# TNO-MPC/protocols.distributed_keygen

Measured on NVIDIA B200. Metric: threshold decrypts/sec (2048-bit N), higher is better.
Workload: dtype u32 limbs (exact integer)

## Files before the change

### protocols/distributed_keygen_b200/csrc/dkg_coop.cuh

```cuda
#pragma once
#include <cuda_runtime.h>
#include <stdint.h>

#include "dkg_coop_params.h"
#include "dkg_mont.cuh"

namespace dkg {

namespace coop {

using sa = uint32_t;
__device__ __forceinline__ sa saddr(const void* p) { return (sa)__cvta_generic_to_shared(p); }

template <int K>
struct NoIO {
  static constexpr int VW = 2;
  struct Prefetch {};
  __device__ __forceinline__ void prefetch_load(const Prefetch&, int, uint32_t (&)[K]) const {}
};

template <int K>
__device__ __forceinline__ void lds(uint32_t (&r)[K], sa p) {
  if constexpr (K % 4 == 0) {
#pragma unroll
// ... 3 lines not shown
  } else {
#pragma unroll
    for (int v = 0; v < K / 2; ++v)
      asm volatile("ld.shared.v2.u32 {%0, %1}, [%2];" : "=r"(r[2 * v]), "=r"(r[2 * v + 1]) : "r"(p + 8u * v) : "memory");
  }
}
template <int K>
__device__ __forceinline__ void sts(sa p, const uint32_t (&r)[K]) {
#pragma unroll
  for (int v = 0; v < K / 2; ++v)
    asm volatile("st.shared.v2.u32 [%0], {%1, %2};" :: "r"(p + 8u * v), "r"(r[2 * v]), "r"(r[2 * v + 1]) : "memory");
}
__device__ __forceinline__ uint32_t lds1(sa p) {
  uint32_t v;
  asm volatile("ld.shared.u32 %0, [%1];" : "=r"(v) : "r"(p) : "memory");
  return v;
}

struct LanePlan {
  int d, i0, i1, p0, p1, p2, rounds, ndiag;
  __device__ __forceinline__ void load(const CoopPlanTable& t, int lane) {
    d = t.d[lane]; i0 = t.i0[lane]; i1 = t.i1[lane];
    p0 = t.partner[0][lane]; p1 = t.partner[1][lane]; p2 = t.partner[2][lane];
    rounds = t.rounds; ndiag = t.ndiag;
  }
};

template <int K, int NS>
__device__ __forceinline__ void product(uint32_t (&e)[NS][2 * K + 2], const LanePlan& lp, int lane, const sa (&X)[NS],
                                        const sa (&Y)[NS], const sa (&X2)[NS], const sa (&Y2)[NS]) {
  ColAcc<K> a[NS];
#pragma unroll
  for (int s = 0; s < NS; ++s) {
#pragma unroll
    for (int p = 0; p < 2 * K + 2; ++p) e[s][p] = 0;
    acc_load<K>(a[s], e[s]);
    acc_clear_side<K>(a[s]);
  }
  const NoIO<K> io;
  const typename NoIO<K>::Prefetch pf;
  for (int i = lp.i0; i < lp.i1; ++i) {
    uint32_t xb[NS][K], yb[NS][K];
    const uint32_t ox = (uint32_t)(i * K * 4), oy = (uint32_t)((lp.d - i) * K * 4);
#pragma unroll
    for (int s = 0; s < NS; ++s) { lds<K>(xb[s], X[s] + ox); lds<K>(yb[s], Y[s] + oy); }
#pragma unroll
    for (int s = 0; s < NS; ++s) block_mac<K>(a[s], xb[s], yb[s], io, pf);
#pragma unroll
    for (int s = 0; s < NS; ++s) {
      if (X2[s] != 0) {
        lds<K>(xb[s], X2[s] + ox);
        lds<K>(yb[s], Y2[s] + oy);
        block_mac<K>(a[s], xb[s], yb[s], io, pf);
      }
    }
  }
  __syncwarp();
#pragma unroll
  for (int s = 0; s < NS; ++s) acc_merge<K>(a[s], e[s]);
  for (int r = 0; r < lp.rounds; ++r) {
    const int src = r == 0 ? lp.p0 : (r == 1 ? lp.p1 : lp.p2);
    const int from = src >= 0 ? src : lane;
    const uint32_t m = src >= 0 ? 0xffffffffu : 0u;
#pragma unroll
    for (int s = 0; s < NS; ++s) {
      uint32_t t[2 * K + 2];
#pragma unroll
      for (int k = 0; k < 2 * K + 2; ++k) t[k] = __shfl_sync(kCoopFull, e[s][k], from) & m;
      add_cc(e[s][0], t[0]);
#pragma unroll
// ... 729 lines not shown
```

### protocols/distributed_keygen_b200/csrc/dkg_modexp.cuh

```cuda
#pragma once
#include <cuda_runtime.h>
#include "dkg_mont.cuh"
#include "dkg_modexp_params.h"

namespace dkg {

template <int K> struct VecSel { using T = uint2; static constexpr int VW = 2; };
#define DKG_VEC4(K_) template <> struct VecSel<K_> { using T = uint4; static constexpr int VW = 4; };
DKG_VEC4(4) DKG_VEC4(8) DKG_VEC4(12) DKG_VEC4(16) DKG_VEC4(20) DKG_VEC4(24) DKG_VEC4(28) DKG_VEC4(32)
#undef DKG_VEC4

__device__ __forceinline__ void unpack(const uint4& v, uint32_t* r) { r[0] = v.x; r[1] = v.y; r[2] = v.z; r[3] = v.w; }
__device__ __forceinline__ void unpack(const uint2& v, uint32_t* r) { r[0] = v.x; r[1] = v.y; }
__device__ __forceinline__ void pack(uint4& v, const uint32_t* r) { v = make_uint4(r[0], r[1], r[2], r[3]); }
__device__ __forceinline__ void pack(uint2& v, const uint32_t* r) { v = make_uint2(r[0], r[1]); }

__device__ __forceinline__ void lds_vec(uint4& v, uint32_t saddr) {
  asm volatile("ld.shared.v4.u32 {%0, %1, %2, %3}, [%4];" : "=r"(v.x), "=r"(v.y), "=r"(v.z), "=r"(v.w) : "r"(saddr) : "memory");
}
__device__ __forceinline__ void lds_vec(uint2& v, uint32_t saddr) {
  asm volatile("ld.shared.v2.u32 {%0, %1}, [%2];" : "=r"(v.x), "=r"(v.y) : "r"(saddr) : "memory");
}
__device__ __forceinline__ void sts_vec(uint32_t saddr, const uint4& v) {
  asm volatile("st.shared.v4.u32 [%0], {%1, %2, %3, %4};" :: "r"(saddr), "r"(v.x), "r"(v.y), "r"(v.z), "r"(v.w) : "memory");
// ... 97 lines not shown
    for (int q = 0; q < KV; q++) { V v; ldg_vec(v, Qg + (size_t)(i * KV + q) * 32); unpack(v, &r[q * VW]); }
  }
  struct Prefetch { const char* base; };
  __device__ __forceinline__ Prefetch prefetch_desc(int kind, int blk) const {
    Prefetch d;
    const bool xkind = kind == PAIR_XX || kind == PAIR_XX2 || kind == PAIR_SX2;
    const bool from_shared = xkind && !x_global();
    const bool none = !(xkind || kind == PAIR_XY || kind == PAIR_NQ || kind == PAIR_SY2);
    unsigned long long sgen;
    const uint32_t sbase = none ? ss : xs;
    asm("cvta.shared.u64 %0, %1;" : "=l"(sgen) : "l"((unsigned long long)(sbase + (uint32_t)((none ? 0 : blk) * KV) * 32u * VB)));
    const V* g = kind == PAIR_XY ? Y : (kind == PAIR_SY2 ? Y2 : ((xkind && x_global()) ? this->xg_get() : Qg));
    const char* gb = reinterpret_cast<const char*>(g + (size_t)(blk * KV) * 32);
    d.base = (from_shared || none) ? reinterpret_cast<const char*>(sgen) : gb;
    return d;
  }
  __device__ __forceinline__ void prefetch_load(const Prefetch& d, int v, uint32_t (&r)[KP]) const {
    V val;
    ld_generic(val, d.base + (size_t)v * 32u * VB);
    unpack(val, &r[v * VW]);
  }
  __device__ __forceinline__ void load_n(int j, uint32_t (&r)[KP]) const {
#pragma unroll
    for (int q = 0; q < KV; q++) { V v; lds_vec(v, ns + (uint32_t)(j * KV + q) * NSTRIDE); unpack(v, &r[q * VW]); }
  }
  __device__ __forceinline__ void load_ninv(uint32_t (&r)[KP]) const {
#pragma unroll
    for (int q = 0; q < KV; q++) { V v; lds_vec(v, nis + (uint32_t)q * NSTRIDE); unpack(v, &r[q * VW]); }
  }
  __device__ __forceinline__ void store_q(int i, const uint32_t (&r)[KP]) const {
#pragma unroll
    for (int q = 0; q < KV; q++) { V v; pack(v, &r[q * VW]); stg_vec(Qg + (size_t)(i * KV + q) * 32, v); }
  }
  __device__ __forceinline__ void store_x(int i, const uint32_t (&r)[KP]) const {
    if (x_global()) {
#pragma unroll
      for (int q = 0; q < KV; q++) { V v; pack(v, &r[q * VW]); stg_vec(this->xg_get() + (size_t)(i * KV + q) * 32, v); }
      return;
    }
#pragma unroll
    for (int q = 0; q < KV; q++) { V v; pack(v, &r[q * VW]); sts_vec(xs + (uint32_t)(i * KV + q) * 32u * VB, v); }
  }
};


template <int VW>
__device__ __forceinline__ int sidx(int l) { return (l / VW) * 32 * VW + (l % VW); }

static __device__ __noinline__ uint32_t* mod_inverse_arrays(uint32_t* pu, uint32_t* pv, uint32_t* px1, uint32_t* px2,
                                                     const uint32_t* Ns, uint32_t n0inv, int Lp, uint32_t* bad_out) {
  uint32_t nz = 0;
  for (int l = 0; l < Lp; ++l) {
    pv[l * 32] = Ns[l];
    px1[l * 32] = (l == 0) ? 1u : 0u;
    px2[l * 32] = 0u;
    nz |= pu[l * 32];
  }
  int len = Lp;
  int guard = 64 * Lp + 64;
  while (nz != 0 && guard-- > 0) {
    uint32_t u0 = pu[0];
    while ((u0 & 1u) == 0) {
      const int tz = u0 ? __ffs(u0) - 1 : 32;
      uint32_t lo = u0;
      for (int l = 0; l < len; ++l) {
        const uint32_t hi = (l + 1 < len) ? pu[(l + 1) * 32] : 0u;
// ... 33 lines not shown
    }
    bool xlt = false;
    for (int l = Lp - 1; l >= 0; --l) {
      const uint32_t a = px1[l * 32], b = px2[l * 32];
      if (a != b) { xlt = a < b; break; }
    }
    const uint32_t addmask = xlt ? 0xffffffffu : 0u;
    int64_t c = 0;
    for (int l = 0; l < Lp; ++l) {
      const int64_t t = (int64_t)px1[l * 32] - (int64_t)px2[l * 32] + (int64_t)(Ns[l] & addmask) + c;
      px1[l * 32] = (uint32_t)t;
      c = t >> 32;
    }
    while (len > 1 && pu[(len - 1) * 32] == 0 && pv[(len - 1) * 32] == 0) --len;
  }
  uint32_t bad = pv[0] ^ 1u;
  for (int l = 1; l < Lp; ++l) bad |= pv[l * 32];
  *bad_out = bad ? 1u : 0u;
  return px2;
}

template <int K, int M>
__device__ uint32_t mod_inverse_lane(uint32_t* X, const uint32_t* Ns, uint32_t n0inv, uint32_t* g) {
  constexpr int VW = VecSel<K>::VW;
  constexpr int Lp = K * M;
  for (int l = 0; l < Lp; ++l) g[l * 32] = X[sidx<VW>(l)];
  uint32_t bad = 0;
  const uint32_t* r = mod_inverse_arrays(g, g + Lp * 32, g + 2 * Lp * 32, g + 3 * Lp * 32, Ns, n0inv, Lp, &bad);
  for (int l = 0; l < Lp; ++l) X[sidx<VW>(l)] = r[l * 32];
  return bad;
}

template <int K, int M, bool PLN, bool SCHED, bool XG>
__device__ __noinline__ void mont_call_rt(const WarpIO<K, M, PLN, SCHED, XG> io, const int mode) {
  mont_mul<K, M>(io, mode);
}
template <int K, int M, int MODE, bool PLN = false, bool SCHED = false, bool XG = false>
__device__ __forceinline__ void mont_call(const WarpIO<K, M, PLN, SCHED, XG>& io) {
  mont_call_rt<K, M, PLN, SCHED, XG>(io, MODE);
}
template <int M>
__device__ __forceinline__ void fill_schedule(uint32_t* tab) {
  const int n = sched_offset<M>(kSchedModes);
  for (int i = threadIdx.x; i < n; i += blockDim.x) tab[i] = sched_entry<M>(i);
}

template <int K, int M>
__global__ void __launch_bounds__(DKG_MAX_THREADS, 1) modexp_fixed_kernel(const ModexpParams p) {
  using V = typename VecSel<K>::T;
  constexpr int VW = VecSel<K>::VW;
  constexpr int Lp = K * M;
  constexpr int LV = Lp / VW;

  extern __shared__ __align__(16) unsigned char smem_raw[];
  uint32_t* Ns32 = reinterpret_cast<uint32_t*>(smem_raw);
  constexpr int UNI = ((Lp + K) * 4 + 15) / 16 * 16;
  const int lane = threadIdx.x & 31, warp = threadIdx.x >> 5, nwarps = blockDim.x >> 5;

  for (int i = threadIdx.x; i < Lp + K; i += blockDim.x) Ns32[i] = p.consts[i];
  __syncthreads();

  V* Xw = reinterpret_cast<V*>(smem_raw + UNI) + (size_t)warp * LV * 32;
  uint32_t* Xw32 = reinterpret_cast<uint32_t*>(Xw);
  const V* Ns = reinterpret_cast<const V*>(Ns32);
  const V* NIs = reinterpret_cast<const V*>(Ns32 + Lp);
  const V* ONEg = reinterpret_cast<const V*>(p.consts + Lp + K + Lp);
  const V* R2rep = reinterpret_cast<const V*>(p.consts + Lp + K + 3 * Lp) + lane;
  const V* ONErep = R2rep + (size_t)LV * 32;

  const unsigned gwarp = blockIdx.x * nwarps + warp;
  uint32_t* scratch32 = p.scratch + (size_t)gwarp * p.scratch_per_warp;
  V* tab = reinterpret_cast<V*>(scratch32);
// ... 116 lines not shown
```

### protocols/distributed_keygen_b200/csrc/dkg_mont.cuh

```cuda
#pragma once
#include "dkg_prims.cuh"

namespace dkg {

enum MontMode { MONT_MUL = 0, MONT_REDC = 1, MONT_SQR = 2, MONT_MUL2S = 3, MONT_MULADD = 4 };

#ifndef DKG_PIPE_BALLAST
#define DKG_PIPE_BALLAST 4096
#endif
DKG_HD uint32_t pipe_ballast(uint32_t a, uint32_t b) {
#if defined(__CUDA_ARCH__)
  float f = __uint_as_float(a);
  const float g = __uint_as_float(b);
#pragma unroll
  for (int q = 0; q < DKG_PIPE_BALLAST; q++) asm volatile("fma.rn.f32 %0, %0, %1, %1;" : "+f"(f) : "f"(g));
  return __float_as_uint(f);
#else
  return a ^ b;
#endif
}

template <int K> constexpr int kpad = K + (K & 1);
template <int K> constexpr int kodd0 = K + 1 - (K & 1);
template <int K> constexpr int kncE = (2 * K - kpad<K>) / 2 + 1;
// ... 22 lines not shown

struct PairDesc {
  int kind, xi, yi;
};

template <int K, class IO>
DKG_HD void block_mac(ColAcc<K>& a, const uint32_t (&x)[kpad<K>], uint32_t (&y)[kpad<K>], const IO& io,
                      const typename IO::Prefetch& pf) {
  static_assert(K >= 4, "K must be >= 4");
  constexpr int VW = IO::VW;
#pragma unroll
  for (int j = 0; j < K; j++) {
    {
      const int i0 = j & 1;
      const int last = ((K - 1 - i0) & 1) ? K - 2 : K - 1;
      mad_cc64(a.E[(i0 + j) / 2], x[i0], y[j]);
#pragma unroll
      for (int i = i0 + 2; i < last; i += 2) madc_cc64(a.E[(i + j) / 2], x[i], y[j]);
      madc_cc64_count(a.E[(last + j) / 2], x[last], y[j], a.CE[(last + j + 2 - kpad<K>) / 2]);
    }
    {
      const int i0 = (j & 1) ^ 1;
      const int last = ((K - 1 - i0) & 1) ? K - 2 : K - 1;
      mad_cc64(a.O[(i0 + j - 1) / 2], x[i0], y[j]);
#pragma unroll
      for (int i = i0 + 2; i < last; i += 2) madc_cc64(a.O[(i + j - 1) / 2], x[i], y[j]);
      madc_cc64_count(a.O[(last + j - 1) / 2], x[last], y[j], a.CO[(last + j + 2 - kodd0<K>) / 2]);
    }
    if ((j + 1) % VW == 0 || j == K - 1) io.prefetch_load(pf, j / VW, y);
  }
}

template <int K>
DKG_HD void acc_merge(ColAcc<K>& a, uint32_t (&e)[2 * K + 2]) {
  uint32_t o[2 * K - 2];
#pragma unroll
  for (int p = 0; p < K + 1; p++) unpack64(a.E[p], e[2 * p], e[2 * p + 1]);
#pragma unroll
  for (int p = 0; p < K - 1; p++) unpack64(a.O[p], o[2 * p], o[2 * p + 1]);
  add_cc(e[1], o[0]);
#pragma unroll
  for (int p = 1; p < 2 * K - 2; p++) addc_cc(e[p + 1], o[p]);
  addc_cc(e[2 * K - 1], 0);
  addc_cc(e[2 * K], 0);
  addc(e[2 * K + 1], 0);
#pragma unroll
  for (int p = K; p <= 2 * K; p++) {
    const bool even = ((p - kpad<K>) & 1) == 0;
    const uint32_t cnt = even ? a.CE[(p - kpad<K>) / 2] : a.CO[(p - kodd0<K>) / 2];
    if (p == K) add_cc(e[p], cnt); else addc_cc(e[p], cnt);
  }
  addc(e[2 * K + 1], 0);
  acc_clear_side<K>(a);
}

template <int K>
DKG_HD void acc_low(const ColAcc<K>& a, uint32_t (&tl)[K]) {
  uint32_t t[kpad<K>], o[kpad<K>];
#pragma unroll
  for (int p = 0; p < (K + 1) / 2; p++) unpack64(a.E[p], t[2 * p], t[2 * p + 1]);
#pragma unroll
  for (int p = 0; p < K / 2; p++) unpack64(a.O[p], o[2 * p], o[2 * p + 1]);
  add_cc(t[1], o[0]);
#pragma unroll
  for (int p = 2; p < K; p++) {
    if (p < K - 1) addc_cc(t[p], o[p - 1]); else addc(t[p], o[p - 1]);
  }
#pragma unroll
  for (int p = 0; p < K; p++) tl[p] = t[p];
}

template <int K>
DKG_HD void acc_load(ColAcc<K>& a, const uint32_t (&e)[2 * K + 2]) {
#pragma unroll
  for (int p = 0; p < K + 1; p++) a.E[p] = pack64(e[2 * p], e[2 * p + 1]);
}

template <int K, int XN>
DKG_HD void block_mul_lo(uint32_t (&r)[kpad<K>], const uint32_t (&x)[XN], const uint32_t (&y)[kpad<K>]) {
  static_assert(XN >= K, "x too short");
  uint32_t E[K + 1], O[K + 1];
#pragma unroll
  for (int i = 0; i < K + 1; i++) { E[i] = 0; O[i] = 0; }
#pragma unroll
  for (int j = 0; j < K; j++) {
    {
      const int i0 = j & 1;
#pragma unroll
      for (int i = i0; i + j <= K - 1; i += 2) {
        const int pos = i + j;
        if (pos <= K - 2) { if (i == i0) mad_cc(E[pos], E[pos + 1], x[i], y[j]); else madc_cc(E[pos], E[pos + 1], x[i], y[j]); }
        else { if (i == i0) mad_lo(E[pos], x[i], y[j]); else madc_lo(E[pos], x[i], y[j]); }
      }
    }
    {
      const int i0 = (j & 1) ^ 1;
#pragma unroll
      for (int i = i0; i + j <= K - 1; i += 2) {
        const int q = i + j - 1;
        if (q + 1 <= K - 2) { if (i == i0) mad_cc(O[q], O[q + 1], x[i], y[j]); else madc_cc(O[q], O[q + 1], x[i], y[j]); }
        else { if (i == i0) mad_lo(O[q], x[i], y[j]); else madc_lo(O[q], x[i], y[j]); }
      }
    }
  }
  r[0] = E[0];
  r[1] = E[1];
  add_cc(r[1], O[0]);
#pragma unroll
  for (int p = 2; p < K - 1; p++) { r[p] = E[p]; addc_cc(r[p], O[p - 1]); }
  r[K - 1] = E[K - 1];
  addc(r[K - 1], O[K - 2]);
  if (K & 1) r[K] = 0;
}

template <int M>
struct ColPlan {
  int lo = 0, span = 0, nxy = 0, nq = 0, total = 0, MODE = 0;
  DKG_HD constexpr ColPlan(int c, int mode) {
    MODE = mode;
    lo = c >= M ? c - M + 1 : 0;
    const int hi = c < M ? c : M - 1;
    span = hi - lo + 1;
    nxy = (MODE == MONT_MUL || MODE == MONT_MUL2S) ? span
          : (MODE == MONT_SQR ? span / 2 + (span & 1) : (MODE == MONT_MULADD ? 2 * span : 0));
    nq = (c < M ? c - 1 : M - 1) - lo + 1;
    total = nxy + nq + (c < M ? 1 : 0);
  }
  DKG_HD constexpr PairDesc at(int c, int t) const {
    PairDesc d{PAIR_NONE, 0, 0};
    if (t < nq) { d.kind = PAIR_NQ; d.yi = lo + t; d.xi = c - d.yi; }
    else if (t < nq + nxy) {
      const int u = t - nq;
      if (MODE == MONT_MULADD && u >= span) { d.kind = PAIR_SY2; d.xi = lo + (u - span); d.yi = c - d.xi; }
      else {
        d.xi = lo + u; d.yi = c - d.xi;
        d.kind = MODE == MONT_SQR ? (d.xi < d.yi ? PAIR_XX2 : PAIR_XX) : (MODE == MONT_MUL2S ? PAIR_SX2 : PAIR_XY);
      }
    } else d.kind = PAIR_QC;
    return d;
  }
};

DKG_HD uint32_t pack_desc(const PairDesc& d) { return (uint32_t)d.kind | ((uint32_t)d.xi << 8) | ((uint32_t)d.yi << 16); }
DKG_HD PairDesc unpack_desc(uint32_t w) {
  PairDesc d;
  d.kind = (int)(w & 0xffu); d.xi = (int)((w >> 8) & 0xffu); d.yi = (int)((w >> 16) & 0xffu);
  return d;
}
constexpr int kSchedModes = 5;
template <int M>
DKG_HD constexpr int sched_words(int mode) {
  int n = 1;
  for (int c = 0; c < 2 * M; ++c) n += ColPlan<M>(c, mode).total;
  return n;
}
template <int M>
DKG_HD constexpr int sched_offset(int mode) {
  int off = 0;
  for (int m = 0; m < mode; ++m) off += sched_words<M>(m);
  return off;
}
template <int M>
DKG_HD uint32_t sched_entry(int i) {
  for (int mode = 0; mode < kSchedModes; ++mode) {
    const int n = sched_words<M>(mode);
    if (i >= n) { i -= n; continue; }
    for (int c = 0; c < 2 * M; ++c) {
      const ColPlan<M> plan(c, mode);
      if (i < plan.total) return pack_desc(plan.at(c, i));
      i -= plan.total;
    }
    break;
  }
  PairDesc none;
  none.kind = PAIR_NONE; none.xi = 0; none.yi = 0;
  return pack_desc(none);
}

template <int K, int M, class IO>
DKG_HD void mont_mul(const IO& io, const int MODE) {
  using Plan = ColPlan<M>;
  ColAcc<K> a;
  uint32_t e[2 * K + 2];
  uint32_t Tc[K + 2];
#pragma unroll
  for (int i = 0; i < K + 2; i++) Tc[i] = 0;
  acc_clear_side<K>(a);

  auto sched = io.sched_begin(IO::SCHED ? sched_offset<M>(MODE) + 1 : 0);
  uint32_t sched_ahead = 0;
  if constexpr (IO::SCHED) sched_ahead = io.sched_word(sched, 0);

  constexpr int KP = kpad<K>;
  uint32_t xb[KP], yb[KP];
  {
    const PairDesc d = Plan(0, MODE).at(0, 0);
    if (d.kind == PAIR_XY) { io.load_x(d.xi, xb); io.load_y(d.yi, yb); }
    else if (d.kind == PAIR_XX) { io.load_x(d.xi, xb); io.load_x(d.yi, yb); }
    else if (d.kind == PAIR_SX2) { io.load_xs2(true, d.xi, xb); io.load_x(d.yi, yb); }
  }

  for (int c = 0; c < 2 * M; ++c) {
    const Plan plan(c, MODE);

#pragma unroll
    for (int p = 0; p < K + 2; p++) e[p] = Tc[p];
#pragma unroll
    for (int p = K + 2; p < 2 * K + 2; p++) e[p] = 0;

    if (MODE == MONT_REDC && c < M) {
      uint32_t tb[KP];
      io.load_x(c, tb);
      add_cc(e[0], tb[0]);
#pragma unroll
      for (int p = 1; p < K; p++) addc_cc(e[p], tb[p]);
#pragma unroll
      for (int p = K; p <= 2 * K; p++) addc_cc(e[p], 0);
      addc(e[2 * K + 1], 0);
    }
    if (MODE == MONT_SQR && (c & 1) == 0 && c >= 2) {
      const int j = c >> 1;
      const uint32_t mask = 0u - (io.x_top_limb(j - 1) >> 31);
      uint32_t tb[KP];
      io.load_x(j, tb);
      add_cc(e[0], tb[0] & mask);
#pragma unroll
      for (int p = 1; p < K; p++) addc_cc(e[p], tb[p] & mask);
#pragma unroll
      for (int p = K; p <= 2 * K; p++) addc_cc(e[p], 0);
      addc(e[2 * K + 1], 0);
    }
    const int t_quot = c < M ? plan.total - 1 : -1;
    int t = 0;
    while (t < plan.total) {
      if (t == 0) acc_load<K>(a, e);
      if (t == t_quot) {
        uint32_t tl[K];
        acc_low<K>(a, tl);
        io.load_ninv(yb);
        block_mul_lo<K>(xb, tl, yb);
        io.store_q(c, xb);
        io.load_n(0, yb);
      }
      int t_end = plan.total;
      if (t < t_quot) t_end = t_quot;
      for (; t < t_end; ++t) {
        PairDesc nx;
        if constexpr (IO::SCHED) {
          nx = unpack_desc(sched_ahead);
          sched = io.sched_next(sched);
          sched_ahead = io.sched_word(sched, 0);
        } else {
          nx.kind = PAIR_NONE; nx.xi = 0; nx.yi = 0;
          if (t + 1 < plan.total) nx = plan.at(c, t + 1);
          else if (c + 1 < 2 * M) {
            const Plan np(c + 1, MODE);
            if (np.total > 0) nx = np.at(c + 1, 0);
          }
        }
        block_mac<K>(a, xb, yb, io, io.prefetch_desc(nx.kind, nx.yi));
        if (nx.kind == PAIR_NQ) io.load_n(nx.xi, xb);
        else if (nx.kind == PAIR_XX2 || nx.kind == PAIR_SX2) io.load_xs2(nx.kind == PAIR_SX2, nx.xi, xb);
        else if (nx.kind != PAIR_QC && nx.kind != PAIR_NONE) io.load_xs(nx.kind == PAIR_SY2, nx.xi, xb);
      }
    }
    if (plan.total > 0) acc_merge<K>(a, e);

    if (c >= M) {
      uint32_t ob[KP];
#pragma unroll
      for (int p = 0; p < K; p++) ob[p] = e[p];
      if (K & 1) ob[K] = 0;
      io.store_x(c - M, ob);
    }
#pragma unroll
    for (int p = 0; p < K + 2; p++) Tc[p] = e[p + K];
  }

  if (io.never()) Tc[0] = pipe_ballast(Tc[0], Tc[1]);
  if (!io.any_lane(Tc[0])) return;
  const uint32_t mask = 0u - Tc[0];
  uint32_t borrow = 0;
  for (int b = 0; b < M; ++b) {
    uint32_t tb[kpad<K>], nb[kpad<K>];
    io.load_x(b, tb);
    io.load_n(b, nb);
#pragma unroll
    for (int p = 0; p < K; p++) {
      const uint64_t d = (uint64_t)tb[p] - (nb[p] & mask) - borrow;
      tb[p] = (uint32_t)d;
      borrow = (uint32_t)(d >> 63);
    }
    io.store_x(b, tb);
  }
}

template <int K, int M, class IO>
DKG_HD uint32_t geq_n(const IO& io) {
  uint32_t borrow = 0;
  for (int b = 0; b < M; ++b) {
    uint32_t xb[kpad<K>], nb[kpad<K>];
    io.load_x(b, xb);
    io.load_n(b, nb);
#pragma unroll
    for (int p = 0; p < K; p++) {
      const uint64_t d = (uint64_t)xb[p] - nb[p] - borrow;
      borrow = (uint32_t)(d >> 63);
    }
  }
  return borrow ^ 1u;
}

template <int K, int M, class IO>
DKG_HD void sub_n_masked(const IO& io, uint32_t mask) {
  uint32_t borrow = 0;
  for (int b = 0; b < M; ++b) {
    uint32_t xb[kpad<K>], nb[kpad<K>];
    io.load_x(b, xb);
    io.load_n(b, nb);
#pragma unroll
    for (int p = 0; p < K; p++) {
      const uint64_t d = (uint64_t)xb[p] - (nb[p] & mask) - borrow;
      xb[p] = (uint32_t)d;
      borrow = (uint32_t)(d >> 63);
    }
    io.store_x(b, xb);
  }
// ... 12 lines not shown
```

### protocols/distributed_keygen_b200/csrc/dkg_nsq.cuh

```cuda
#pragma once
#include "dkg_modexp.cuh"
#include "dkg_nsq_params_fwd.h"

namespace dkg {


template <int K, int M>
__device__ __forceinline__ void pair_fixup(typename VecSel<kpad<K>>::T* Bv, const typename VecSel<kpad<K>>::T* mq,
                                           const uint32_t* Ns, const uint32_t* Dneg) {
  constexpr int KP = kpad<K>;
  using V = typename VecSel<KP>::T;
  constexpr int VW = VecSel<KP>::VW;
  constexpr int LV = KP * M / VW;
  auto is_pad = [](int v, int k) -> bool { return (K & 1) && (v * VW + k) % KP == K; };
  uint32_t carry = 1;
  for (int v = 0; v < LV; ++v) {
    uint32_t bb[VW], mm[VW];
    unpack(Bv[v * 32], bb);
    unpack(mq[(size_t)v * 32], mm);
#pragma unroll
    for (int k = 0; k < VW; ++k) {
      if (is_pad(v, k)) { bb[k] = 0; continue; }
      const uint64_t s = (uint64_t)bb[k] + (uint32_t)~mm[k] + carry;
      bb[k] = (uint32_t)s;
      carry = (uint32_t)(s >> 32);
    }
    V o; pack(o, bb); Bv[v * 32] = o;
  }
  const uint32_t need = carry ^ 1u;
  if (__any_sync(0xffffffffu, need)) {
    const uint32_t mask = 0u - need;
    uint32_t c2 = 0;
    for (int v = 0; v < LV; ++v) {
      uint32_t bb[VW];
      unpack(Bv[v * 32], bb);
#pragma unroll
      for (int k = 0; k < VW; ++k) {
        if (is_pad(v, k)) continue;
        const uint64_t s = (uint64_t)bb[k] + (Dneg[v * VW + k] & mask) + c2;
        bb[k] = (uint32_t)s;
        c2 = (uint32_t)(s >> 32);
      }
      V o; pack(o, bb); Bv[v * 32] = o;
    }
    if (__any_sync(0xffffffffu, c2)) {
      const uint32_t mask2 = 0u - c2;
      uint32_t borrow = 0;
      for (int v = 0; v < LV; ++v) {
        uint32_t bb[VW];
        unpack(Bv[v * 32], bb);
#pragma unroll
        for (int k = 0; k < VW; ++k) {
          if (is_pad(v, k)) continue;
          const uint64_t d = (uint64_t)bb[k] - (Ns[v * VW + k] & mask2) - borrow;
          bb[k] = (uint32_t)d;
          borrow = (uint32_t)(d >> 63);
        }
        V o; pack(o, bb); Bv[v * 32] = o;
      }
    }
  }
}

template <int K, int M, class PairMul>
__device__ __forceinline__ uint32_t pair_invert(typename VecSel<kpad<K>>::T* Aw, typename VecSel<kpad<K>>::T* Bw,
                                                uint32_t* work, const uint32_t* U32, const uint32_t* Nd,
                                                const uint32_t* two_ab, const typename VecSel<kpad<K>>::T* R2Ar,
                                                const typename VecSel<kpad<K>>::T* R2Br, int lane, PairMul&& pair_mul) {
  constexpr int KP = kpad<K>;
  using V = typename VecSel<KP>::T;
  constexpr int VW = VecSel<KP>::VW;
  constexpr int Lp = KP * M, La = K * M, LV = Lp / VW, KVB = KP / VW;
  uint32_t* Aw32 = reinterpret_cast<uint32_t*>(Aw);
  uint32_t* Bw32 = reinterpret_cast<uint32_t*>(Bw);
  uint32_t* pu = work + lane;
  uint32_t* pv = pu + La * 32;
  V* slots = reinterpret_cast<V*>(work + 2 * Lp * 32);
  auto slot_a = [&](int s) -> V* { return slots + (size_t)s * 2 * LV * 32 + lane; };
  auto slot_b = [&](int s) -> V* { return slots + ((size_t)s * 2 + 1) * LV * 32 + lane; };
  auto sidx_of = [&](int l) -> int { const int sl = (l / K) * KP + l % K; return ((sl / VW) * 32 + lane) * VW + sl % VW; };
  for (int v = 0; v < LV; ++v) { slot_a(0)[(size_t)v * 32] = Aw[v * 32 + lane]; slot_b(0)[(size_t)v * 32] = Bw[v * 32 + lane]; }
  for (int l = 0; l < La; ++l) pu[l * 32] = Aw32[sidx_of(l)];
  uint32_t bad = 0;
  const uint32_t* g = mod_inverse_arrays(pu, pv, Aw32 + lane, Bw32 + lane, Nd, U32[Lp], La, &bad);
  if (g != pu) for (int l = 0; l < La; ++l) pu[l * 32] = g[l * 32];
  {
    const V zero = V();
    for (int v = 0; v < LV; ++v) { Aw[v * 32 + lane] = zero; Bw[v * 32 + lane] = zero; }
  }
  for (int l = 0; l < La; ++l) Aw32[sidx_of(l)] = pu[l * 32];
  pair_mul(R2Ar, R2Br);
  pair_mul(R2Ar, R2Br);
  for (int v = 0; v < LV; ++v) { slot_a(1)[(size_t)v * 32] = Aw[v * 32 + lane]; slot_b(1)[(size_t)v * 32] = Bw[v * 32 + lane]; }
  pair_mul(slot_a(0), slot_b(0));
// ... 49 lines not shown
  const uint32_t* Ns32 = U32;
  const uint32_t* Dneg = U32 + Lp + KP;
  const uint32_t* Nd = U32 + 2 * Lp + KP;

  V* Aw = reinterpret_cast<V*>(smem_raw + UNI) + (size_t)warp * (BG ? 1 : 2) * LV * 32;
  uint32_t* Aw32 = reinterpret_cast<uint32_t*>(Aw);
  const V* Cg = reinterpret_cast<const V*>(p.consts + 2 * Lp + KP);
  const V* ONEA = Cg + 2 * LV, *ONEB = Cg + 3 * LV;
  const V* Crep = Cg + 6 * LV + lane;
  const V* R2Ar = Crep, *R2Br = Crep + (size_t)LV * 32, *ONEAr = Crep + (size_t)2 * LV * 32,
          *ONEBr = Crep + (size_t)3 * LV * 32,
          *PLAIN1r = Crep + (size_t)4 * LV * 32, *ZEROr = Crep + (size_t)5 * LV * 32;
  const uint32_t* two_ab = p.consts + (2 * Lp + KP) + 6 * Lp + 6 * Lp * 32;

  const unsigned gwarp = blockIdx.x * nwarps + warp;
  uint32_t* scratch32 = p.scratch + (size_t)gwarp * p.scratch_per_warp;
  V* tab = reinterpret_cast<V*>(scratch32);
  V* Qg = reinterpret_cast<V*>(scratch32 + p.scratch_q_offset);
  V* Bw = BG ? Qg + LV * 32 : Aw + LV * 32;
  uint32_t* Bw32 = reinterpret_cast<uint32_t*>(Bw);

  const uint32_t a_s = (uint32_t)__cvta_generic_to_shared(Aw + lane);
  const uint32_t b_s = BG ? 0u : (uint32_t)__cvta_generic_to_shared(Bw + lane);
  WarpIO<K, M, false, true, BG> io;
  io.sched_s = (uint32_t)__cvta_generic_to_shared(smem_raw + UNI0);
  io.ns = (uint32_t)__cvta_generic_to_shared(Ns32);
  io.nis = (uint32_t)__cvta_generic_to_shared(Ns32 + Lp);
  io.Qg = Qg + lane;

  auto pair_mul = [&](const V* c, const V* d) {
    io.xs = b_s; io.ss = a_s; io.Y = c; io.Y2 = d;
    if constexpr (BG) io.xg = Bw + lane;
    mont_call<K, M, MONT_MULADD, false, true, BG>(io);
    io.xs = a_s;
    if constexpr (BG) io.xg = nullptr;
    mont_call<K, M, MONT_MUL, false, true, BG>(io);
    pair_fixup<K, M>(Bw + lane, Qg + lane, Ns32, Dneg);
  };
  auto pair_sqr = [&]() {
    io.xs = b_s; io.ss = a_s;
    if constexpr (BG) io.xg = Bw + lane;
    mont_call<K, M, MONT_MUL2S, false, true, BG>(io);
    io.xs = a_s;
    if constexpr (BG) io.xg = nullptr;
    mont_call<K, M, MONT_SQR, false, true, BG>(io);
    pair_fixup<K, M>(Bw + lane, Qg + lane, Ns32, Dneg);
  };

  const unsigned long long ngroups = (p.count + 31ull) / 32ull;
  for (;;) {
    unsigned int g = 0;
    if (lane == 0) g = atomicAdd(p.counter, 1u);
    g = __shfl_sync(0xffffffffu, g, 0);
    if (g >= ngroups) break;
    const unsigned long long first = (unsigned long long)g * 32ull;
    const int cnt = (int)((p.count - first) < 32ull ? (p.count - first) : 32ull);

    for (int r = 0; r < 32; ++r) {
      const uint32_t* row = p.pairs_in + (first + (unsigned long long)r) * (unsigned long long)(2 * La);
      for (int l = lane; l < Lp; l += 32) {
        const int i = ((l / VW) * 32 + r) * VW + (l % VW);
        const int src = (l / KP) * K + (l % KP);
        const bool pad = (l % KP) >= K;
        Aw32[i] = pad ? 0u : ((r < cnt) ? row[src] : (l == 0 ? 1u : 0u));
        Bw32[i] = (pad || r >= cnt) ? 0u : row[La + src];
      }
    }
    __syncwarp();

    pair_mul(R2Ar, R2Br);
    uint32_t st = 0;
    if (p.negative)
      st = pair_invert<K, M>(Aw, Bw, scratch32 + p.inv_slot * (unsigned long long)(2 * Lp * 32), U32, Nd, two_ab, R2Ar, R2Br, lane, pair_mul);
    if (p.nops == 0) {
      for (int v = 0; v < LV; ++v) { Aw[v * 32 + lane] = ONEA[v]; Bw[v * 32 + lane] = ONEB[v]; }
    } else {
      const int tn = p.tab_entries;
      auto tab_a = [&](int k) -> V* { return tab + (size_t)k * 2 * LV * 32 + lane; };
      auto tab_b = [&](int k) -> V* { return tab + ((size_t)k * 2 + 1) * LV * 32 + lane; };
// ... 98 lines not shown

  V* Aw = reinterpret_cast<V*>(smem_raw + UNI) + (size_t)warp * (BG ? 1 : 2) * LV * 32;
  uint32_t* Aw32 = reinterpret_cast<uint32_t*>(Aw);
  const V* Cg = reinterpret_cast<const V*>(p.consts + 2 * Lp + KP);
  const V* Crep = Cg + 6 * LV + lane;
  const V* R2Ar = Crep, *R2Br = Crep + (size_t)LV * 32, *ONEAr = Crep + (size_t)2 * LV * 32,
          *ONEBr = Crep + (size_t)3 * LV * 32,
          *PLAIN1r = Crep + (size_t)4 * LV * 32, *ZEROr = Crep + (size_t)5 * LV * 32;
  const uint32_t* two_ab = p.consts + (2 * Lp + KP) + 6 * Lp + 6 * Lp * 32;

  const unsigned gwarp = blockIdx.x * nwarps + warp;
  uint32_t* scratch32 = p.scratch + (size_t)gwarp * p.scratch_per_warp;
  V* slots = reinterpret_cast<V*>(scratch32);
  V* Qg = reinterpret_cast<V*>(scratch32 + p.scratch_q_offset);
  V* Bw = BG ? Qg + LV * 32 : Aw + LV * 32;
  uint32_t* Bw32 = reinterpret_cast<uint32_t*>(Bw);
  const int D = 1 << p.wbits;
  auto slot_a = [&](int s) -> V* { return slots + (size_t)s * 2 * LV * 32 + lane; };
  auto slot_b = [&](int s) -> V* { return slots + ((size_t)s * 2 + 1) * LV * 32 + lane; };
  const int CUR = p.nparties * D, ACC = CUR + 1;

  const uint32_t a_s = (uint32_t)__cvta_generic_to_shared(Aw + lane);
  const uint32_t b_s = BG ? 0u : (uint32_t)__cvta_generic_to_shared(Bw + lane);
  WarpIO<K, M, false, true, BG> io;
  io.sched_s = (uint32_t)__cvta_generic_to_shared(smem_raw + UNI0);
  io.ns = (uint32_t)__cvta_generic_to_shared(Ns32);
  io.nis = (uint32_t)__cvta_generic_to_shared(Ns32 + Lp);
  io.Qg = Qg + lane;

  auto pair_mul = [&](const V* c, const V* d) {
    io.xs = b_s; io.ss = a_s; io.Y = c; io.Y2 = d;
    if constexpr (BG) io.xg = Bw + lane;
    mont_call<K, M, MONT_MULADD, false, true, BG>(io);
    io.xs = a_s;
    if constexpr (BG) io.xg = nullptr;
    mont_call<K, M, MONT_MUL, false, true, BG>(io);
    pair_fixup<K, M>(Bw + lane, Qg + lane, Ns32, Dneg);
  };
  auto pair_sqr = [&]() {
    io.xs = b_s; io.ss = a_s;
    if constexpr (BG) io.xg = Bw + lane;
    mont_call<K, M, MONT_MUL2S, false, true, BG>(io);
    io.xs = a_s;
    if constexpr (BG) io.xg = nullptr;
    mont_call<K, M, MONT_SQR, false, true, BG>(io);
    pair_fixup<K, M>(Bw + lane, Qg + lane, Ns32, Dneg);
  };
  auto park = [&](int s) {
    V* da = slot_a(s); V* db = slot_b(s);
#pragma unroll 5
    for (int v = 0; v < LV; ++v) { da[(size_t)v * 32] = Aw[v * 32 + lane]; db[(size_t)v * 32] = Bw[v * 32 + lane]; }
  };
  auto fetch = [&](int s) {
    const V* sa = slot_a(s); const V* sb = slot_b(s);
#pragma unroll 5
    for (int v = 0; v < LV; ++v) { Aw[v * 32 + lane] = sa[(size_t)v * 32]; Bw[v * 32 + lane] = sb[(size_t)v * 32]; }
  };

  const unsigned long long ngroups = (p.count + 31ull) / 32ull;
  for (;;) {
    unsigned int g = 0;
    if (lane == 0) g = atomicAdd(p.counter, 1u);
    g = __shfl_sync(0xffffffffu, g, 0);
    if (g >= ngroups) break;
    const unsigned long long first = (unsigned long long)g * 32ull;
    const int cnt = (int)((p.count - first) < 32ull ? (p.count - first) : 32ull);

    for (int r = 0; r < 32; ++r) {
      const uint32_t* row = p.pairs_in + (first + (unsigned long long)r) * (unsigned long long)(2 * La);
      for (int l = lane; l < Lp; l += 32) {
        const int i = ((l / VW) * 32 + r) * VW + (l % VW);
        const int src = (l / KP) * K + (l % KP);
        const bool pad = (l % KP) >= K;
        Aw32[i] = pad ? 0u : ((r < cnt) ? row[src] : (l == 0 ? 1u : 0u));
        Bw32[i] = (pad || r >= cnt) ? 0u : row[La + src];
      }
    }
    __syncwarp();
    pair_mul(R2Ar, R2Br);
// ... 60 lines not shown
```

Measured before the change: 60420.

## Fold pair fixup subtraction into Montgomery quotient loop and carry accumulator directly

The B-minus-Q correction that pair_fixup did in a separate pass is now folded into mont_mul: each quotient block is subtracted from B via a not-add with a running carry right after it is computed, and only the rare tail correction remains outside. The column loop also stops materialising a 2K+2 limb e[] array per column, keeping the running carry in Tc and merging it into the accumulator low limbs directly. This removes a full extra read-modify-write sweep over B and Q per pair operation and some register shuffling. In exchange mont_mul gains extra global/shared traffic inside the quotient step and more complex carry handling, which may raise register pressure.

Result: no change. 60750 (median of 6 runs) (+0.6%).

```diff
diff --git a/protocols/distributed_keygen_b200/csrc/dkg_coop.cuh b/protocols/distributed_keygen_b200/csrc/dkg_coop.cuh
--- a/protocols/distributed_keygen_b200/csrc/dkg_coop.cuh
+++ b/protocols/distributed_keygen_b200/csrc/dkg_coop.cuh
@@ -59,10 +59,7 @@
   ColAcc<K> a[NS];
 #pragma unroll
   for (int s = 0; s < NS; ++s) {
-#pragma unroll
-    for (int p = 0; p < 2 * K + 2; ++p) e[s][p] = 0;
-    acc_load<K>(a[s], e[s]);
-    acc_clear_side<K>(a[s]);
+    acc_clear<K>(a[s]);
   }
   const NoIO<K> io;
   const typename NoIO<K>::Prefetch pf;
diff --git a/protocols/distributed_keygen_b200/csrc/dkg_modexp.cuh b/protocols/distributed_keygen_b200/csrc/dkg_modexp.cuh
--- a/protocols/distributed_keygen_b200/csrc/dkg_modexp.cuh
+++ b/protocols/distributed_keygen_b200/csrc/dkg_modexp.cuh
@@ -153,6 +153,16 @@
 #pragma unroll
     for (int q = 0; q < KV; q++) { V v; pack(v, &r[q * VW]); stg_vec(Qg + (size_t)(i * KV + q) * 32, v); }
   }
+  V* fb = nullptr;
+  __device__ __forceinline__ bool fold_b() const { return fb != nullptr; }
+  __device__ __forceinline__ void load_b(int i, uint32_t (&r)[KP]) const {
+#pragma unroll
+    for (int q = 0; q < KV; q++) unpack(fb[(size_t)(i * KV + q) * 32], &r[q * VW]);
+  }
+  __device__ __forceinline__ void store_b(int i, const uint32_t (&r)[KP]) const {
+#pragma unroll
+    for (int q = 0; q < KV; q++) pack(fb[(size_t)(i * KV + q) * 32], &r[q * VW]);
+  }
   __device__ __forceinline__ void store_x(int i, const uint32_t (&r)[KP]) const {
     if (x_global()) {
 #pragma unroll
@@ -252,12 +262,12 @@
 }
 
 template <int K, int M, bool PLN, bool SCHED, bool XG>
-__device__ __noinline__ void mont_call_rt(const WarpIO<K, M, PLN, SCHED, XG> io, const int mode) {
-  mont_mul<K, M>(io, mode);
+__device__ __noinline__ uint32_t mont_call_rt(const WarpIO<K, M, PLN, SCHED, XG> io, const int mode) {
+  return mont_mul<K, M>(io, mode);
 }
 template <int K, int M, int MODE, bool PLN = false, bool SCHED = false, bool XG = false>
-__device__ __forceinline__ void mont_call(const WarpIO<K, M, PLN, SCHED, XG>& io) {
-  mont_call_rt<K, M, PLN, SCHED, XG>(io, MODE);
+__device__ __forceinline__ uint32_t mont_call(const WarpIO<K, M, PLN, SCHED, XG>& io) {
+  return mont_call_rt<K, M, PLN, SCHED, XG>(io, MODE);
 }
 template <int M>
 __device__ __forceinline__ void fill_schedule(uint32_t* tab) {
diff --git a/protocols/distributed_keygen_b200/csrc/dkg_mont.cuh b/protocols/distributed_keygen_b200/csrc/dkg_mont.cuh
--- a/protocols/distributed_keygen_b200/csrc/dkg_mont.cuh
+++ b/protocols/distributed_keygen_b200/csrc/dkg_mont.cuh
@@ -78,6 +78,13 @@
 }
 
 template <int K>
+DKG_HD void acc_clear(ColAcc<K>& a) {
+#pragma unroll
+  for (int i = 0; i < K + 1; i++) a.E[i] = 0;
+  acc_clear_side<K>(a);
+}
+
+template <int K>
 DKG_HD void acc_merge(ColAcc<K>& a, uint32_t (&e)[2 * K + 2]) {
   uint32_t o[2 * K - 2];
 #pragma unroll
@@ -101,7 +108,26 @@
 }
 
 template <int K>
-DKG_HD void acc_low(const ColAcc<K>& a, uint32_t (&tl)[K]) {
+DKG_HD void acc_merge_carry(ColAcc<K>& a, uint32_t (&Tc)[K + 2], uint32_t (&lo)[kpad<K>]) {
+  uint32_t e[2 * K + 2];
+  acc_merge<K>(a, e);
+  add_cc(e[0], Tc[0]);
+#pragma unroll
+  for (int p = 1; p < K + 2; p++) addc_cc(e[p], Tc[p]);
+#pragma unroll
+  for (int p = K + 2; p < 2 * K + 1; p++) addc_cc(e[p], 0);
+  addc(e[2 * K + 1], 0);
+#pragma unroll
+  for (int p = 0; p < K; p++) lo[p] = e[p];
+  if (K & 1) lo[K] = 0;
+#pragma unroll
+  for (int p = 0; p < K + 2; p++) Tc[p] = e[p + K];
+#pragma unroll
+  for (int p = 0; p < K + 1; p++) a.E[p] = 0;
+}
+
+template <int K>
+DKG_HD void acc_low(const ColAcc<K>& a, const uint32_t (&Tc)[K + 2], uint32_t (&tl)[K]) {
   uint32_t t[kpad<K>], o[kpad<K>];
 #pragma unroll
   for (int p = 0; p < (K + 1) / 2; p++) unpack64(a.E[p], t[2 * p], t[2 * p + 1]);
@@ -112,14 +138,12 @@
   for (int p = 2; p < K; p++) {
     if (p < K - 1) addc_cc(t[p], o[p - 1]); else addc(t[p], o[p - 1]);
   }
+  add_cc(t[0], Tc[0]);
+#pragma unroll
+  for (int p = 1; p < K - 1; p++) addc_cc(t[p], Tc[p]);
+  addc(t[K - 1], Tc[K - 1]);
 #pragma unroll
   for (int p = 0; p < K; p++) tl[p] = t[p];
-}
-
-template <int K>
-DKG_HD void acc_load(ColAcc<K>& a, const uint32_t (&e)[2 * K + 2]) {
-#pragma unroll
-  for (int p = 0; p < K + 1; p++) a.E[p] = pack64(e[2 * p], e[2 * p + 1]);
 }
 
 template <int K, int XN>
@@ -158,6 +182,20 @@
   addc(r[K - 1], O[K - 2]);
   if (K & 1) r[K] = 0;
 }
+
+template <int K>
+DKG_HD uint32_t block_add_not(uint32_t (&b)[kpad<K>], const uint32_t (&q)[kpad<K>], uint32_t carry) {
+  add_cc(carry, 0xffffffffu);
+#pragma unroll
+  for (int p = 0; p < K; p++) addc_cc(b[p], ~q[p]);
+  uint32_t out = 0;
+  addc(out, 0);
+  if (K & 1) b[K] = 0;
+  return out;
+}
+
+template <class IO, class = void> struct FoldsB { static constexpr bool value = false; };
+template <class IO> struct FoldsB<IO, decltype((void)&IO::fold_b)> { static constexpr bool value = true; };
 
 template <int M>
 struct ColPlan {
@@ -224,14 +262,14 @@
 }
 
 template <int K, int M, class IO>
-DKG_HD void mont_mul(const IO& io, const int MODE) {
+DKG_HD uint32_t mont_mul(const IO& io, const int MODE) {
   using Plan = ColPlan<M>;
   ColAcc<K> a;
-  uint32_t e[2 * K + 2];
   uint32_t Tc[K + 2];
 #pragma unroll
   for (int i = 0; i < K + 2; i++) Tc[i] = 0;
-  acc_clear_side<K>(a);
+  acc_clear<K>(a);
+  uint32_t fold_carry = 1;
 
   auto sched = io.sched_begin(IO::SCHED ? sched_offset<M>(MODE) + 1 : 0);
   uint32_t sched_ahead = 0;
@@ -249,43 +287,43 @@
   for (int c = 0; c < 2 * M; ++c) {
     const Plan plan(c, MODE);
 
-#pragma unroll
-    for (int p = 0; p < K + 2; p++) e[p] = Tc[p];
-#pragma unroll
-    for (int p = K + 2; p < 2 * K + 2; p++) e[p] = 0;
-
     if (MODE == MONT_REDC && c < M) {
       uint32_t tb[KP];
       io.load_x(c, tb);
-      add_cc(e[0], tb[0]);
-#pragma unroll
-      for (int p = 1; p < K; p++) addc_cc(e[p], tb[p]);
-#pragma unroll
-      for (int p = K; p <= 2 * K; p++) addc_cc(e[p], 0);
-      addc(e[2 * K + 1], 0);
+      add_cc(Tc[0], tb[0]);
+#pragma unroll
+      for (int p = 1; p < K; p++) addc_cc(Tc[p], tb[p]);
+      addc_cc(Tc[K], 0);
+      addc(Tc[K + 1], 0);
     }
     if (MODE == MONT_SQR && (c & 1) == 0 && c >= 2) {
       const int j = c >> 1;
       const uint32_t mask = 0u - (io.x_top_limb(j - 1) >> 31);
       uint32_t tb[KP];
       io.load_x(j, tb);
-      add_cc(e[0], tb[0] & mask);
-#pragma unroll
-      for (int p = 1; p < K; p++) addc_cc(e[p], tb[p] & mask);
-#pragma unroll
-      for (int p = K; p <= 2 * K; p++) addc_cc(e[p], 0);
-      addc(e[2 * K + 1], 0);
+      add_cc(Tc[0], tb[0] & mask);
+#pragma unroll
+      for (int p = 1; p < K; p++) addc_cc(Tc[p], tb[p] & mask);
+      addc_cc(Tc[K], 0);
+      addc(Tc[K + 1], 0);
     }
     const int t_quot = c < M ? plan.total - 1 : -1;
     int t = 0;
     while (t < plan.total) {
-      if (t == 0) acc_load<K>(a, e);
       if (t == t_quot) {
         uint32_t tl[K];
-        acc_low<K>(a, tl);
+        acc_low<K>(a, Tc, tl);
         io.load_ninv(yb);
         block_mul_lo<K>(xb, tl, yb);
         io.store_q(c, xb);
+        if constexpr (FoldsB<IO>::value) {
+          if (io.fold_b()) {
+            uint32_t bb[KP];
+            io.load_b(c, bb);
+            fold_carry = block_add_not<K>(bb, xb, fold_carry);
+            io.store_b(c, bb);
+          }
+        }
         io.load_n(0, yb);
       }
       int t_end = plan.total;
@@ -310,21 +348,21 @@
         else if (nx.kind != PAIR_QC && nx.kind != PAIR_NONE) io.load_xs(nx.kind == PAIR_SY2, nx.xi, xb);
       }
     }
-    if (plan.total > 0) acc_merge<K>(a, e);
-
-    if (c >= M) {
-      uint32_t ob[KP];
-#pragma unroll
-      for (int p = 0; p < K; p++) ob[p] = e[p];
+    uint32_t ob[KP];
+    if (plan.total > 0) {
+      acc_merge_carry<K>(a, Tc, ob);
+    } else {
+#pragma unroll
+      for (int p = 0; p < K; p++) ob[p] = Tc[p];
       if (K & 1) ob[K] = 0;
-      io.store_x(c - M, ob);
-    }
-#pragma unroll
-    for (int p = 0; p < K + 2; p++) Tc[p] = e[p + K];
+#pragma unroll
+      for (int p = 0; p < K + 2; p++) Tc[p] = p + K < K + 2 ? Tc[p + K] : 0u;
+    }
+    if (c >= M) io.store_x(c - M, ob);
   }
 
   if (io.never()) Tc[0] = pipe_ballast(Tc[0], Tc[1]);
-  if (!io.any_lane(Tc[0])) return;
+  if (!io.any_lane(Tc[0])) return fold_carry;
   const uint32_t mask = 0u - Tc[0];
   uint32_t borrow = 0;
   for (int b = 0; b < M; ++b) {
@@ -339,6 +377,7 @@
     }
     io.store_x(b, tb);
   }
+  return fold_carry;
 }
 
 template <int K, int M, class IO>
diff --git a/protocols/distributed_keygen_b200/csrc/dkg_nsq.cuh b/protocols/distributed_keygen_b200/csrc/dkg_nsq.cuh
--- a/protocols/distributed_keygen_b200/csrc/dkg_nsq.cuh
+++ b/protocols/distributed_keygen_b200/csrc/dkg_nsq.cuh
@@ -4,6 +4,49 @@
 
 namespace dkg {
 
+
+template <int K, int M>
+__device__ __forceinline__ void pair_fixup_tail(typename VecSel<kpad<K>>::T* Bv, uint32_t carry, const uint32_t* Ns,
+                                                const uint32_t* Dneg) {
+  constexpr int KP = kpad<K>;
+  using V = typename VecSel<KP>::T;
+  constexpr int VW = VecSel<KP>::VW;
+  constexpr int LV = KP * M / VW;
+  auto is_pad = [](int v, int k) -> bool { return (K & 1) && (v * VW + k) % KP == K; };
+  const uint32_t need = carry ^ 1u;
+  if (__any_sync(0xffffffffu, need)) {
+    const uint32_t mask = 0u - need;
+    uint32_t c2 = 0;
+    for (int v = 0; v < LV; ++v) {
+      uint32_t bb[VW];
+      unpack(Bv[v * 32], bb);
+#pragma unroll
+      for (int k = 0; k < VW; ++k) {
+        if (is_pad(v, k)) continue;
+        const uint64_t s = (uint64_t)bb[k] + (Dneg[v * VW + k] & mask) + c2;
+        bb[k] = (uint32_t)s;
+        c2 = (uint32_t)(s >> 32);
+      }
+      V o; pack(o, bb); Bv[v * 32] = o;
+    }
+    if (__any_sync(0xffffffffu, c2)) {
+      const uint32_t mask2 = 0u - c2;
+      uint32_t borrow = 0;
+      for (int v = 0; v < LV; ++v) {
+        uint32_t bb[VW];
+        unpack(Bv[v * 32], bb);
+#pragma unroll
+        for (int k = 0; k < VW; ++k) {
+          if (is_pad(v, k)) continue;
+          const uint64_t d = (uint64_t)bb[k] - (Ns[v * VW + k] & mask2) - borrow;
+          bb[k] = (uint32_t)d;
+          borrow = (uint32_t)(d >> 63);
+        }
+        V o; pack(o, bb); Bv[v * 32] = o;
+      }
+    }
+  }
+}
 
 template <int K, int M>
 __device__ __forceinline__ void pair_fixup(typename VecSel<kpad<K>>::T* Bv, const typename VecSel<kpad<K>>::T* mq,
@@ -27,39 +70,7 @@
     }
     V o; pack(o, bb); Bv[v * 32] = o;
   }
-  const uint32_t need = carry ^ 1u;
-  if (__any_sync(0xffffffffu, need)) {
-    const uint32_t mask = 0u - need;
-    uint32_t c2 = 0;
-    for (int v = 0; v < LV; ++v) {
-      uint32_t bb[VW];
-      unpack(Bv[v * 32], bb);
-#pragma unroll
-      for (int k = 0; k < VW; ++k) {
-        if (is_pad(v, k)) continue;
-        const uint64_t s = (uint64_t)bb[k] + (Dneg[v * VW + k] & mask) + c2;
-        bb[k] = (uint32_t)s;
-        c2 = (uint32_t)(s >> 32);
-      }
-      V o; pack(o, bb); Bv[v * 32] = o;
-    }
-    if (__any_sync(0xffffffffu, c2)) {
-      const uint32_t mask2 = 0u - c2;
-      uint32_t borrow = 0;
-      for (int v = 0; v < LV; ++v) {
-        uint32_t bb[VW];
-        unpack(Bv[v * 32], bb);
-#pragma unroll
-        for (int k = 0; k < VW; ++k) {
-          if (is_pad(v, k)) continue;
-          const uint64_t d = (uint64_t)bb[k] - (Ns[v * VW + k] & mask2) - borrow;
-          bb[k] = (uint32_t)d;
-          borrow = (uint32_t)(d >> 63);
-        }
-        V o; pack(o, bb); Bv[v * 32] = o;
-      }
-    }
-  }
+  pair_fixup_tail<K, M>(Bv, carry, Ns, Dneg);
 }
 
 template <int K, int M, class PairMul>
@@ -175,19 +186,21 @@
     io.xs = b_s; io.ss = a_s; io.Y = c; io.Y2 = d;
     if constexpr (BG) io.xg = Bw + lane;
     mont_call<K, M, MONT_MULADD, false, true, BG>(io);
-    io.xs = a_s;
+    io.xs = a_s; io.fb = Bw + lane;
     if constexpr (BG) io.xg = nullptr;
-    mont_call<K, M, MONT_MUL, false, true, BG>(io);
-    pair_fixup<K, M>(Bw + lane, Qg + lane, Ns32, Dneg);
+    const uint32_t carry = mont_call<K, M, MONT_MUL, false, true, BG>(io);
+    io.fb = nullptr;
+    pair_fixup_tail<K, M>(Bw + lane, carry, Ns32, Dneg);
   };
   auto pair_sqr = [&]() {
     io.xs = b_s; io.ss = a_s;
     if constexpr (BG) io.xg = Bw + lane;
     mont_call<K, M, MONT_MUL2S, false, true, BG>(io);
-    io.xs = a_s;
+    io.xs = a_s; io.fb = Bw + lane;
     if constexpr (BG) io.xg = nullptr;
-    mont_call<K, M, MONT_SQR, false, true, BG>(io);
-    pair_fixup<K, M>(Bw + lane, Qg + lane, Ns32, Dneg);
+    const uint32_t carry = mont_call<K, M, MONT_SQR, false, true, BG>(io);
+    io.fb = nullptr;
+    pair_fixup_tail<K, M>(Bw + lane, carry, Ns32, Dneg);
   };
 
   const unsigned long long ngroups = (p.count + 31ull) / 32ull;
@@ -352,19 +365,21 @@
     io.xs = b_s; io.ss = a_s; io.Y = c; io.Y2 = d;
     if constexpr (BG) io.xg = Bw + lane;
     mont_call<K, M, MONT_MULADD, false, true, BG>(io);
-    io.xs = a_s;
+    io.xs = a_s; io.fb = Bw + lane;
     if constexpr (BG) io.xg = nullptr;
-    mont_call<K, M, MONT_MUL, false, true, BG>(io);
-    pair_fixup<K, M>(Bw + lane, Qg + lane, Ns32, Dneg);
+    const uint32_t carry = mont_call<K, M, MONT_MUL, false, true, BG>(io);
+    io.fb = nullptr;
+    pair_fixup_tail<K, M>(Bw + lane, carry, Ns32, Dneg);
   };
   auto pair_sqr = [&]() {
     io.xs = b_s; io.ss = a_s;
     if constexpr (BG) io.xg = Bw + lane;
     mont_call<K, M, MONT_MUL2S, false, true, BG>(io);
-    io.xs = a_s;
+    io.xs = a_s; io.fb = Bw + lane;
     if constexpr (BG) io.xg = nullptr;
-    mont_call<K, M, MONT_SQR, false, true, BG>(io);
-    pair_fixup<K, M>(Bw + lane, Qg + lane, Ns32, Dneg);
+    const uint32_t carry = mont_call<K, M, MONT_SQR, false, true, BG>(io);
+    io.fb = nullptr;
+    pair_fixup_tail<K, M>(Bw + lane, carry, Ns32, Dneg);
   };
   auto park = [&](int s) {
     V* da = slot_a(s); V* db = slot_b(s);
```
